# ygina/sidekick

Hardware: AMD Instinct MI355X
Metric: quACK encode identifiers/s (device-resident), u32 ids, threshold t=32 (higher is better)
Workload: dtype u32; 1 GPU; encode 1e+09 u32 ids per GPU at t=32, device-resident; ids_per_gpu=1000000000, global_ids=1000000000, threshold=32, bits=32, seed=0x5eed0002, parallelism=shard1, collectives=single

## Files before the change

### sidekick_amd/csrc/api.hip

```cpp
#include <string.h>

#include <algorithm>
#include <chrono>
#include <thread>
#include <vector>

#include "ctx.h"
#include "field.h"

using namespace qk;

#pragma clang diagnostic ignored "-Wunused-value"
#pragma clang diagnostic ignored "-Wunused-result"

namespace qk {

QK_WARM_KERNEL(api)

hipStream_t pick_stream(qk_ctx *ctx, void *stream) {
    (void)ctx;
    return (hipStream_t)stream;
}

int scratch_acquire(qk_ctx *ctx, hipStream_t s) {
// ... 336 lines not shown
template int root_test_begin<uint32_t>(qk_ctx *, const RtPlan<uint32_t> &, const uint32_t *, uint32_t,
                                       const uint32_t *, size_t, int, uint32_t, hipStream_t);
template int root_test_begin<uint64_t>(qk_ctx *, const RtPlan<uint64_t> &, const uint64_t *, uint32_t,
                                       const uint64_t *, size_t, int, uint64_t, hipStream_t);
template int root_test_finish<uint32_t>(qk_ctx *, const RtPlan<uint32_t> &, const uint32_t *, uint32_t,
                                        const uint32_t *, size_t, int, uint32_t, hipStream_t, std::vector<uint64_t> &,
                                        uint64_t &);
template int root_test_finish<uint64_t>(qk_ctx *, const RtPlan<uint64_t> &, const uint64_t *, uint32_t,
                                        const uint64_t *, size_t, int, uint64_t, hipStream_t, std::vector<uint64_t> &,
                                        uint64_t &);

template <typename T>
static int root_test_scan_k(qk_ctx *ctx, const T *coeffs, uint32_t d, const T *d_log, size_t n, int use_stop,
                            T stop_value, hipStream_t s, std::vector<uint64_t> &h, uint64_t &stop) {
    std::vector<T> r(d);
    uint32_t k = 0;
    int rc;
    if constexpr (sizeof(T) == 4) rc = qk_u32_roots(coeffs, d, r.data(), d, &k);
    else rc = qk_u64_roots(coeffs, d, r.data(), d, &k);
    if (rc) return rc;
    RtScanSet set;
    std::vector<T> tab;
    if (!rt_scan_table<T>(r.data(), k, set, tab, true) || set.words * sizeof(T) > RT_KTAB_BYTES) return 1;
    if (int e = ensure_hits(ctx, 4096, s)) return e;
    uint64_t *hs = ctx->h_small;
    if (!ctx->rt_bases_valid) {
        QK_HIP_TRY(hipMemsetAsync(ctx->d_small + SMALL_KT, 0, 4 * sizeof(uint64_t), s));
        ctx->rt_hbase = ctx->rt_sbase = 0;
    }
    if (!ctx->rt_slots_clean) {
        std::fill(hs + SMALL_HITPF, hs + SMALL_WORDS, ~0ull);
        hs[SMALL_OVF] = 0;
    }
    ctx->rt_slots_clean = false;
    const uint64_t gen = ++ctx->rt_gen;
    if (int e = launch_root_scan_k<T>(ctx, tab, set, d_log, n, use_stop, stop_value, ctx->d_hits,
                                      (uint64_t)ctx->hits_cap, ctx->d_small + SMALL_KT, ctx->h_small_dev + SMALL_NHITS,
                                      ctx->rt_hbase, ctx->rt_sbase, ctx->d_small + RT_DONE, gen, s)) {
        ctx->rt_bases_valid = false;
        return e;
    }
    ctx->rt_bases_valid = true;
    const volatile uint64_t *done = hs + SMALL_DONE;
    for (unsigned spin = 0;; ++spin) {
        if (*done == gen) break;
        if ((spin & 63) == 63) {
            const hipError_t q = hipStreamQuery(s);
            if (q != hipSuccess && q != hipErrorNotReady) {
                ctx->rt_bases_valid = false;
                return QK_E_HIP;
            }
            if (q == hipSuccess) {
                if (*done == gen) break;
                QK_HIP_TRY(hipMemsetAsync(ctx->d_small + RT_DONE, 0, (SMALL_DEV_WORDS - RT_DONE) * sizeof(uint64_t), s));
                break;
            }
        }
        if (spin >= 200000) std::this_thread::sleep_for(std::chrono::microseconds(5));
    }
    std::atomic_thread_fence(std::memory_order_acquire);
    if (hs[SMALL_OVF]) {
        ctx->rt_bases_valid = false;
        return 1;
    }
    uint64_t c = 0;
    while (c < SMALL_HITPF_N && hs[SMALL_HITPF + c] != ~0ull) ++c;
    uint64_t st = ~0ull, ns = 0;
    for (uint32_t q = 0; q < RT_NSTOP; ++q) {
        st = std::min(st, hs[SMALL_STOPS + q]);
        ns += hs[SMALL_STOPS + q] != ~0ull;
    }
    ctx->rt_hbase += c;
    ctx->rt_sbase += ns;
    h.assign(hs + SMALL_HITPF, hs + SMALL_HITPF + c);
    std::fill(hs + SMALL_HITPF, hs + SMALL_HITPF + c, ~0ull);
    std::fill(hs + SMALL_STOPS, hs + SMALL_WORDS, ~0ull);
    ctx->rt_slots_clean = true;
    std::sort(h.begin(), h.end());
    stop = use_stop ? std::min<uint64_t>(st, (uint64_t)n) : (uint64_t)n;
    return QK_OK;
}

template <typename T>
static int root_test_impl(qk_ctx *ctx, const T *coeffs, uint32_t d, const T *d_log, size_t n, int use_stop,
                          T stop_value, uint64_t *hits, size_t cap, size_t *n_hits, void *stream,
                          uint64_t *stop_index = nullptr) {
    if (!ctx || !n_hits || (d && !coeffs) || (n && !d_log)) return QK_E_INVAL;
    *n_hits = 0;
    if (stop_index) *stop_index = n;
    if (n == 0) return QK_OK;
    if (d == 0) {
        if (!stop_index || !use_stop) return QK_OK;
    }
    if (d > QK_MAX_THRESHOLD) return QK_E_THRESHOLD;
    if (!is_device_ptr(d_log)) return QK_E_INVAL;
    std::lock_guard<std::mutex> g(ctx->mu);
    QK_HIP_TRY(hipSetDevice(ctx->device));
    hipStream_t s = pick_stream(ctx, stream);
    std::vector<uint64_t> h;
    uint64_t stop = n;
    int ov = 1;
    if (ctx->knobs.rt_karg && rt_use_scan<T>(ctx, d, n)) {
        ov = root_test_scan_k<T>(ctx, coeffs, d, d_log, n, use_stop, stop_value, s, h, stop);
        if (ov < 0) return ov;
    }
    if (ov) {
        RtPlan<T> plan;
// ... 105 lines not shown
int qk_ctx_set_profiling(qk_ctx *ctx, int on) {
    if (!ctx) return QK_E_INVAL;
    std::lock_guard<std::mutex> g(ctx->mu);
    ctx->profiling = on != 0;
    return QK_OK;
}

int qk_ctx_kernel_stats(qk_ctx *ctx, double *total_ms, uint64_t *launches) {
    if (!ctx || !total_ms || !launches) return QK_E_INVAL;
    std::lock_guard<std::mutex> g(ctx->mu);
    double tot = 0;
    uint64_t cnt = 0;
    int rc = QK_OK;
    for (auto &pr : ctx->prof_pending) {
        if (hipEventSynchronize(pr.second) != hipSuccess) rc = QK_E_HIP;
        float ms = 0;
        if (hipEventElapsedTime(&ms, pr.first, pr.second) == hipSuccess) { tot += ms; ++cnt; }
        ctx->ev_pool.push_back(pr.first);
        ctx->ev_pool.push_back(pr.second);
    }
    ctx->prof_pending.clear();
    *total_ms = tot;
    *launches = cnt;
    return rc;
}

int qk_ctx_trim(qk_ctx *ctx) {
    if (!ctx) return QK_E_INVAL;
    std::lock_guard<std::mutex> g(ctx->mu);
    if (ctx->retired.empty()) return QK_OK;
    QK_HIP_TRY(hipSetDevice(ctx->device));
    int rc = QK_OK;
    for (void *r : ctx->retired)
        if (hipFree(r) != hipSuccess) rc = QK_E_HIP;
    ctx->retired.clear();
    return rc;
}

int qk_ctx_set_grid(qk_ctx *ctx, uint32_t blocks) {
    if (!ctx) return QK_E_INVAL;
    ctx->grid_override = blocks;
    return QK_OK;
}

int qk_ctx_set_knob(qk_ctx *ctx, const char *name, int64_t value) {
    if (!ctx || !name) return QK_E_INVAL;
    struct K {
        const char *name;
        int qk_knobs::*field;
        int64_t lo, hi;
    };
    static const K table[] = {
        {"grid_mult", &qk_knobs::grid_mult, 1, 8},
        {"flow_hist", &qk_knobs::flow_hist, 0, 1 << 20},
        {"flow_byslot", &qk_knobs::flow_byslot, 0, 2},
        {"root_test", &qk_knobs::root_test, 0, 2},
        {"comm_fault", &qk_knobs::comm_fault, 0, 1 << 20},
        {"comm_delay_ms", &qk_knobs::comm_delay_ms, 0, 600000},
        {"rt_karg", &qk_knobs::rt_karg, 0, 1},
    };
    for (const K &k : table)
        if (strcmp(k.name, name) == 0) {
            if (value < k.lo || value > k.hi) return QK_E_INVAL;
            std::lock_guard<std::mutex> g(ctx->mu);
            ctx->knobs.*(k.field) = (int)value;
            return QK_OK;
        }
    return QK_E_INVAL;
}

__global__ void k_clock_probe(uint64_t *out, uint64_t ticks) {
    const uint64_t c0 = __builtin_amdgcn_s_memtime(), r0 = __builtin_amdgcn_s_memrealtime();
    uint64_t c1, r1;
    do {
        __builtin_amdgcn_s_sleep(32);
        c1 = __builtin_amdgcn_s_memtime();
        r1 = __builtin_amdgcn_s_memrealtime();
    } while (r1 - r0 < ticks);
    if (threadIdx.x == 0) {
        out[0] = c1 - c0;
        out[1] = r1 - r0;
    }
}

int qk_clock_probe(qk_ctx *ctx, uint32_t microseconds, uint64_t *d_out, void *stream) {
    if (!ctx || !d_out || !microseconds || microseconds > 10000000u) return QK_E_INVAL;
    if (!is_device_ptr(d_out)) return QK_E_INVAL;
    QK_HIP_TRY(hipSetDevice(ctx->device));
    hipLaunchKernelGGL(k_clock_probe, dim3(1), dim3(64), 0, (hipStream_t)stream, d_out, (uint64_t)microseconds * 100);
    QK_HIP_TRY(hipGetLastError());
    return QK_OK;
}

int qk_host_alloc(size_t bytes, void **out) {
    if (!out) return QK_E_INVAL;
    if (hipHostMalloc(out, bytes, hipHostMallocDefault) != hipSuccess) { *out = nullptr; return QK_E_NOMEM; }
    return QK_OK;
}
int qk_host_free(void *p) {
    if (p && hipHostFree(p) != hipSuccess) return QK_E_HIP;
    return QK_OK;
}

int qk_u32_encode_device_async(qk_ctx *ctx, const uint32_t *d_ids, size_t n, uint32_t t, uint64_t *d_partial,
                               void *stream) {
    if (!ctx || !d_partial || (n && !d_ids)) return QK_E_INVAL;
// ... 157 lines not shown
```

### sidekick_amd/csrc/bsgs.h

```cpp
#pragma once
#include <hip/hip_runtime.h>
#include <stdint.h>

#include "field.h"

namespace qk {
namespace bsgs {

constexpr int BLOCK = 256;
constexpr int WAVES = BLOCK / 64;

__device__ __forceinline__ uint64_t shfl_xor_u64(uint64_t v, int m) {
    const uint32_t lo = __shfl_xor((int)(uint32_t)v, m, 64);
    const uint32_t hi = __shfl_xor((int)(uint32_t)(v >> 32), m, 64);
    return ((uint64_t)hi << 32) | lo;
}

#define QK_MAC4V(P0, P1, P2, P3)                                                                       \
    "v_mad_u64_u32 %0, " P0 ", %8, %9, %0\n\t"                                                         \
    "v_mad_u64_u32 %1, " P1 ", %8, %10, %1\n\t"                                                        \
    "v_mad_u64_u32 %2, " P2 ", %8, %11, %2\n\t"                                                        \
    "v_mad_u64_u32 %3, " P3 ", %8, %12, %3\n\t"                                                        \
    "v_addc_co_u32_e64 %4, " P0 ", %4, 0, " P0 "\n\t"                                                  \
    "v_addc_co_u32_e64 %5, " P1 ", %5, 0, " P1 "\n\t"                                                  \
// ... 576 lines not shown
            nxc = *pc;
        }
        four<C>(S, w, base, c, &xo);
        if constexpr (XO) {
            *po = xo;
            po += nthr;
        }
    }
    for (; it < tmax; ++it) {
        const uint4 w = nxt, c = nxc;
        const bool cur = p < vend;
        p += nthr;
        nxt = make_uint4(0, 0, 0, 0);
        if (p < vend) nxt = *p;
        if constexpr (XI) {
            pc += nthr;
            if (p < vend) nxc = *pc;
        }
        four<C>(S, w, base, c, &xo);
        if constexpr (XO) {
            if (cur) *po = xo;
            po += nthr;
        }
        (void)cur;
    }
    const uint64_t tail0 = h + (nbody << 2);
    const uint32_t tid = wave_s * 64u + __lane_id();
    gtid = (((uint64_t)gb_hi << 32) | gb_lo) + tid;
    {
        const bool in = gtid < h;
        uint32_t xn = 0;
        one<C>(S, in ? ids[gtid] : 0u, base, XI && in ? xin[gtid] : 0u, &xn);
        if (XO && in) xout[gtid] = xn;
    }
    {
        const bool in = gtid < n - tail0;
        uint32_t xn = 0;
        one<C>(S, in ? ids[tail0 + gtid] : 0u, base, XI && in ? xin[tail0 + gtid] : 0u, &xn);
        if (XO && in) xout[tail0 + gtid] = xn;
    }

    finish<C>(S, T, out, tid);
}

template <class C>
__device__ __forceinline__ void body(const uint32_t *__restrict__ ids, uint64_t n, uint32_t head, uint32_t T,
                                     uint64_t *__restrict__ partials, uint32_t base = 0,
                                     const uint32_t *xin = nullptr, uint32_t *xout = nullptr) {
    body_gen<C>(
        ids, n, head, T, (uint64_t)blockIdx.x * BLOCK + threadIdx.x, (uint64_t)gridDim.x * BLOCK,
        [=](uint32_t m, uint64_t s) { partials[(size_t)m * gridDim.x + blockIdx.x] = s; }, base, xin, xout);
}

}
}
```

### sidekick_amd/csrc/ctx.h

```cpp
#pragma once
#include <hip/hip_runtime.h>

#include <atomic>
#include <mutex>
#include <vector>

#include "quack_hip.h"

struct qk_knobs {
    int grid_mult = 3;
    int flow_hist = 32;
    int flow_byslot = 0;
    int root_test = 0;
    int comm_fault = 0;
    int rt_karg = 1;
    int comm_delay_ms = 0;
};

struct qk_ctx {
    int device = 0;
    int num_cus = 256;
    int max_threads_per_cu = 2048;
    uint32_t max_blocks_per_cu(uint32_t block) const { return (uint32_t)max_threads_per_cu / block; }
    hipStream_t stream = nullptr;
    hipStream_t copy_stream = nullptr;
    uint32_t grid_override = 0;
    qk_knobs knobs;

    void *d_scratch = nullptr;
    size_t scratch_bytes = 0;
    uint64_t *d_small = nullptr;
    uint64_t *h_small = nullptr;
    uint64_t *h_small_dev = nullptr;
    uint64_t rt_hbase = 0, rt_sbase = 0;
    bool rt_bases_valid = false;
    bool rt_slots_clean = false;
    int rt_occ_k[2] = {0, 0};
    uint64_t rt_gen = 0;
    uint64_t *d_hits = nullptr;
    size_t hits_cap = 0;

    void *d_flow[3] = {nullptr, nullptr, nullptr};
    size_t flow_bytes[3] = {0, 0, 0};
    size_t flow_hint = 0;
    void *h_items = nullptr;
    void *h_items_dev = nullptr;
    size_t h_items_bytes = 0;

    void *h_stage[2] = {nullptr, nullptr};
    void *d_stage[2] = {nullptr, nullptr};
    size_t stage_bytes = 0;
    hipEvent_t stage_ev[2] = {nullptr, nullptr};

    bool profiling = false;
    std::vector<std::pair<hipEvent_t, hipEvent_t>> prof_pending;
    std::vector<hipEvent_t> ev_pool;

    hipEvent_t scratch_ev = nullptr;
    bool scratch_ev_valid = false;
    hipEvent_t flow_ev[3] = {nullptr, nullptr, nullptr};
    uint64_t *h_flow = nullptr;

    std::vector<void *> retired;

    std::mutex mu;
};

#define QK_HIP_TRY(expr)                                                                           \
    do {                                                                                           \
        hipError_t _e = (expr);                                                                    \
        if (_e != hipSuccess) return QK_E_HIP;                                                     \
    } while (0)

namespace qk {

constexpr size_t SMALL_WORDS = 4096;
constexpr size_t RT_C = 4;
constexpr size_t SMALL_NHITS = 3072;
constexpr size_t SMALL_STOP = 3073;
constexpr size_t SMALL_OVF = 3074;
constexpr size_t SMALL_DONE = 3075;
constexpr size_t SMALL_HITPF = 3076;
constexpr uint32_t RT_NSTOP = 16;
constexpr size_t SMALL_STOPS = SMALL_WORDS - RT_NSTOP;
constexpr size_t SMALL_HITPF_N = SMALL_STOPS - SMALL_HITPF;
constexpr size_t RT_STOP0 = SMALL_STOPS - SMALL_NHITS;
constexpr size_t SMALL_KT = SMALL_WORDS - 8;
constexpr uint32_t RT_DONE_GROUPS = 32;
constexpr size_t RT_DONE = SMALL_WORDS;
constexpr size_t SMALL_DEV_WORDS = RT_DONE + 16 * (RT_DONE_GROUPS + 1);

#define QK_WARM_KERNEL(name)                                                                                     \
    __global__ void k_warm_##name(int *p) {                                                                      \
        if (p) p[threadIdx.x] = 0;                                                                               \
    }                                                                                                            \
    int warm_##name(hipStream_t s) {                                                                             \
        hipLaunchKernelGGL(k_warm_##name, dim3(1), dim3(64), 0, s, nullptr);                                     \
        return hipGetLastError() == hipSuccess ? QK_OK : QK_E_HIP;                                               \
    }
int warm_api(hipStream_t s);
int warm_encode(hipStream_t s);
int warm_decode(hipStream_t s);
int warm_packets(hipStream_t s);
int warm_flows(hipStream_t s);
int warm_segments(hipStream_t s);
int warm_comm(hipStream_t s);

hipStream_t pick_stream(qk_ctx *ctx, void *stream);
int scratch_acquire(qk_ctx *ctx, hipStream_t s);
int scratch_release(qk_ctx *ctx, hipStream_t s);
int ensure_scratch(qk_ctx *ctx, size_t bytes, hipStream_t s);
int ensure_hits(qk_ctx *ctx, size_t cap, hipStream_t s);
int ensure_flow(qk_ctx *ctx, int which, size_t bytes, hipStream_t s);
int ensure_stage(qk_ctx *ctx, size_t bytes);
int ensure_items(qk_ctx *ctx, size_t bytes);
bool is_device_ptr(const void *p);
hipEvent_t prof_begin(qk_ctx *ctx, hipStream_t s);
void prof_end(qk_ctx *ctx, hipStream_t s, hipEvent_t begin);

int launch_encode_u32(qk_ctx *ctx, const uint32_t *d_ids, size_t n, uint32_t t, uint64_t *d_partial,
                      hipStream_t s);
int launch_encode_u64(qk_ctx *ctx, const uint64_t *d_ids, size_t n, uint32_t t, uint64_t *d_partial,
                      hipStream_t s);
int launch_encode_u32_acc(qk_ctx *ctx, const uint32_t *d_ids, size_t n, uint32_t t,
                          uint64_t *d_partial, hipStream_t s);
int launch_encode_u64_acc(qk_ctx *ctx, const uint64_t *d_ids, size_t n, uint32_t t,
                          uint64_t *d_partial, hipStream_t s);

int launch_root_test_u32(qk_ctx *ctx, const uint32_t *d_c, uint32_t d, const uint32_t *log, size_t n,
                         int use_stop, uint32_t stop_value, uint64_t *hits, uint64_t cap, uint64_t *counters,
                         hipStream_t s);
int launch_finalize_powers_u32(const uint64_t *partials, uint32_t nblocks, uint32_t T, uint64_t *out,
                               hipStream_t s);
bool rt64_use_bsgs(const qk_ctx *ctx, uint32_t d);
constexpr uint32_t RT_SCAN_MAXD = 256;
size_t rt64_bsgs_table(const uint64_t *coeffs, uint32_t d, uint64_t *out);
int launch_root_test_u64(qk_ctx *ctx, const uint64_t *d_c, uint32_t d, const uint64_t *log, size_t n,
                         int use_stop, uint64_t stop_value, uint64_t *hits, uint64_t cap, uint64_t *counters,
                         hipStream_t s);

struct RtScanSet {
    uint32_t S = 1, words = 0, m1 = 1, m2 = 1, shift = 28;
};
// ... 30 lines not shown
```

### sidekick_amd/csrc/encode.hip

```cpp
#include "ctx.h"
#include "field.h"
#include "bsgs.h"
#include "bsgs64.h"

#ifndef QK_BSGS_SG_T32
#define QK_BSGS_SG_T32 8
#endif
#ifndef QK_BSGS_ROW0
#define QK_BSGS_ROW0 1
#endif
#ifndef QK_BSGS_FOLD
#define QK_BSGS_FOLD 1
#endif

namespace qk {

QK_WARM_KERNEL(encode)

constexpr int BLOCK = 256;
constexpr int WAVES = BLOCK / 64;

__device__ __forceinline__ uint64_t shfl_xor_u64(uint64_t v, int m) {
    const uint32_t lo = __shfl_xor((int)(uint32_t)v, m, 64);
    const uint32_t hi = __shfl_xor((int)(uint32_t)(v >> 32), m, 64);
    return ((uint64_t)hi << 32) | lo;
}


template <int K>
__device__ __forceinline__ void chain32(uint64_t (&acc)[K], uint32_t start, uint32_t step) {
    const uint32_t step5 = times5_32(step);
    uint64_t t = start;
#pragma unroll
    for (int k = 0; k < K; ++k) {
        acc[k] += t;
        if (k + 1 < K) t = tstep32p(t, step, step5, 0u);
    }
}

template <int K>
__device__ __forceinline__ void chain32x4(uint64_t (&acc)[K], uint4 w) {
    const uint32_t x0 = canon32(w.x), x1 = canon32(w.y), x2 = canon32(w.z), x3 = canon32(w.w);
    const uint32_t f0 = times5_32(x0), f1 = times5_32(x1), f2 = times5_32(x2), f3 = times5_32(x3);
    uint64_t t0 = x0, t1 = x1, t2 = x2, t3 = x3;
#pragma unroll
    for (int k = 0; k < K; ++k) {
        acc[k] += t0;
        acc[k] += t1;
        acc[k] += t2;
        acc[k] += t3;
        if (k + 1 < K) {
            t0 = tstep32p(t0, x0, f0, 0u);
            t1 = tstep32p(t1, x1, f1, 0u);
            t2 = tstep32p(t2, x2, f2, 0u);
            t3 = tstep32p(t3, x3, f3, 0u);
        }
    }
}

template <int NB, int NA, int SG, int PRIO = 1>
__global__ __launch_bounds__(BLOCK, (NB * NA == 32 ? 5 : NB * NA > 64 ? 2 : NB * NA > 40 ? 3 : 4)) void k_encode_u32_bsgs(const uint32_t *__restrict__ ids,
                                                                                  uint64_t n, uint32_t head,
                                                                                  uint32_t T,
                                                                                  uint64_t *__restrict__ partials) {
    bsgs::body<bsgs::Cfg<NB, NA, SG, QK_BSGS_ROW0, QK_BSGS_FOLD, false, false, 0, false, PRIO ? 4 : 0>>(ids, n, head,
                                                                                                        T, partials);
}


template <int SG, int PRIO = 1>
__global__ __launch_bounds__(BLOCK, 2) void k_encode_u32_bsgs_x80(const uint32_t *__restrict__ ids, uint64_t n,
                                                                 uint32_t head, uint32_t T,
                                                                 uint64_t *__restrict__ partials,
                                                                 const uint32_t *xin,
                                                                 uint32_t *xout) {
    (void)xin;
    bsgs::body<bsgs::Cfg<8, 10, SG, 1, 1, false, false, 2, false, PRIO ? 4 : 0>>(ids, n, head, T, partials, 0, nullptr,
                                                                                 xout);
}

template <int NA, int SG, int XC = 0, int PRIO = 1>
__global__ __launch_bounds__(BLOCK, (NA > 6 ? 2 : NA > 5 ? 3 : 4)) void k_encode_u32_bsgs_off(
    const uint32_t *__restrict__ ids, uint64_t n, uint32_t head, uint32_t T, uint32_t base,
    uint64_t *__restrict__ partials, const uint32_t *xin, uint32_t *xout) {
    bsgs::body<bsgs::Cfg<8, NA, SG, 1, 1, false, true, XC, false, PRIO ? 4 : 0>>(ids, n, head, T, partials, base, xin,
                                                                                 xout);
}

template <int G>
__device__ __forceinline__ void group_powers32(uint32_t x, int j, uint32_t &start, uint32_t &step) {
    uint32_t b = x, r = 1;
    const uint32_t e = (uint32_t)j + 1;
#pragma unroll
    for (int bit = 0; (1 << bit) <= G; ++bit) {
        const uint32_t rb = mul32_lazy(r, b);
        r = ((e >> bit) & 1) ? rb : r;
        if ((1 << bit) < G) b = mul32_lazy(b, b);
    }
    start = r;
    step = canon32(b);
}

template <int G, int K, typename Fold>
__device__ __forceinline__ void block_store(const uint64_t (&acc)[K], uint32_t T, uint64_t *partials,
                                            uint64_t *sm, Fold fold) {
    const int lane = threadIdx.x & 63, wave = threadIdx.x >> 6;
#pragma unroll
    for (int k = 0; k < K; ++k) {
        uint64_t v = fold(acc[k]);
#pragma unroll
        for (int off = 32; off >= G; off >>= 1) v += shfl_xor_u64(v, off);
        if (lane < G) sm[wave * (G * K) + lane + k * G] = v;
    }
    __syncthreads();
    for (uint32_t m = threadIdx.x; m < T; m += BLOCK) {
        uint64_t s = 0;
#pragma unroll
        for (int w = 0; w < WAVES; ++w) s += sm[w * (G * K) + m];
        partials[(size_t)m * gridDim.x + blockIdx.x] = s;
    }
}
// ... 358 lines not shown
                                                                          uint64_t *xout) {
    (void)head;
    bsgs64::body<10, F ? 3 : 0, 16, 0, 0, false, true, 1, 2, bsgs64::NB, F ? 3 : 0>(ids, n, T, partials, 0, nullptr,
                                                                                 xout);
}

template <int NA, int XC = 0, int F = 1>
__global__ __launch_bounds__(bsgs64::BLOCK, 4) void k_encode_u64_bsgs_off(const uint64_t *__restrict__ ids,
                                                                          uint64_t n, uint32_t head, uint32_t T,
                                                                          uint32_t base,
                                                                          uint64_t *__restrict__ partials,
                                                                          const uint64_t *xin,
                                                                          uint64_t *xout) {
    (void)head;
    bsgs64::body<NA, F ? 3 : 0, 16, 0, 0, true, true, 1, XC, bsgs64::NB, F ? 3 : 0>(ids, n, T, partials, base, xin,
                                                                                     xout);
}

template <typename KernelT>
static uint32_t grid_for(qk_ctx *ctx, KernelT kern, uint64_t units, uint32_t per_block, int mult = 0) {
    if (ctx->grid_override) return ctx->grid_override;
    int occ = 0;
    if (hipOccupancyMaxActiveBlocksPerMultiprocessor(&occ, kern, BLOCK, 0) != hipSuccess || occ < 1) occ = 1;
    const uint64_t full = (uint64_t)ctx->num_cus * (uint64_t)occ * (uint64_t)(mult > 0 ? mult : ctx->knobs.grid_mult);
    uint64_t need = (units + per_block - 1) / per_block;
    if (need < 1) need = 1;
    return (uint32_t)(need < full ? need : full);
}

static uint32_t grid_cap(const qk_ctx *ctx, uint64_t units, uint32_t per_block, int mult = 0) {
    if (ctx->grid_override) return ctx->grid_override;
    const uint64_t full = (uint64_t)ctx->num_cus * (uint64_t)ctx->max_blocks_per_cu(BLOCK) *
                          (uint64_t)(mult > 0 ? mult : ctx->knobs.grid_mult);
    uint64_t need = (units + per_block - 1) / per_block;
    if (need < 1) need = 1;
    return (uint32_t)(need < full ? need : full);
}

template <typename IdT, typename KernelT, typename FinT>
static int run_encode(qk_ctx *ctx, KernelT kern, FinT fin, uint32_t GK, uint32_t words_per_power,
                      const IdT *d_ids, size_t n, uint32_t head, uint32_t T, uint64_t units,
                      uint32_t per_block, uint64_t *d_partial, int accumulate, hipStream_t s, int mult = 0) {
    const uint32_t nb = grid_for(ctx, kern, units, per_block, mult);
    const size_t need = (size_t)nb * words_per_power * GK * sizeof(uint64_t);
    int rc = ensure_scratch(ctx, need, s);
    if (rc) return rc;
    uint64_t *partials = (uint64_t *)ctx->d_scratch;
    rc = scratch_acquire(ctx, s);
    if (rc) return rc;
    hipEvent_t e0 = prof_begin(ctx, s);
    hipLaunchKernelGGL(kern, dim3(nb), dim3(BLOCK), 0, s, d_ids, (uint64_t)n, head, T, partials);
    prof_end(ctx, s, e0);
    QK_HIP_TRY(hipGetLastError());
    hipLaunchKernelGGL(fin, dim3(T), dim3(BLOCK), 0, s, partials, nb, T, d_ids, (uint64_t)n, d_partial,
                       accumulate);
    QK_HIP_TRY(hipGetLastError());
    return scratch_release(ctx, s);
}

int launch_finalize_powers_u32(const uint64_t *partials, uint32_t nblocks, uint32_t T, uint64_t *out,
                               hipStream_t s) {
    hipLaunchKernelGGL(k_finalize_u32_pass, dim3(T), dim3(BLOCK), 0, s, partials, nblocks, T,
                       (const uint32_t *)nullptr, (uint64_t)0, out, (uint64_t *)nullptr, 0);
    return hipGetLastError() == hipSuccess ? QK_OK : QK_E_HIP;
}

template <int KIND, class KernelT>
static int run_pass(qk_ctx *ctx, KernelT kern, uint32_t GK, const uint32_t *d_ids, size_t n,
                    uint32_t head, uint32_t Tp, uint32_t base, uint64_t *out, uint64_t *meta, int acc,
                    hipStream_t s, const uint32_t *xin = nullptr, uint32_t *xout = nullptr) {
    const uint32_t nb = grid_for(ctx, kern, (n + 3) / 4, BLOCK, 1);
    if (int rc = ensure_scratch(ctx, (size_t)nb * GK * sizeof(uint64_t), s)) return rc;
    uint64_t *partials = (uint64_t *)ctx->d_scratch;
    if (int rc = scratch_acquire(ctx, s)) return rc;
    hipEvent_t e0 = prof_begin(ctx, s);
    if constexpr (KIND == 1)
        hipLaunchKernelGGL(kern, dim3(nb), dim3(BLOCK), 0, s, d_ids, (uint64_t)n, head, Tp, base, partials, xin,
                           xout);
    else if constexpr (KIND == 2)
        hipLaunchKernelGGL(kern, dim3(nb), dim3(BLOCK), 0, s, d_ids, (uint64_t)n, head, Tp, partials, xin, xout);
    else
        hipLaunchKernelGGL(kern, dim3(nb), dim3(BLOCK), 0, s, d_ids, (uint64_t)n, head, Tp, partials);
    prof_end(ctx, s, e0);
    QK_HIP_TRY(hipGetLastError());
    hipLaunchKernelGGL(k_finalize_u32_pass, dim3(Tp), dim3(BLOCK), 0, s, partials, nb, Tp, d_ids, (uint64_t)n, out,
                       meta, acc);
    QK_HIP_TRY(hipGetLastError());
    return scratch_release(ctx, s);
}


static int enc32_passes_chunk(qk_ctx *ctx, const uint32_t *ids, size_t n, uint32_t head, uint32_t T, uint64_t *out,
                              int acc, hipStream_t s) {
    const uint32_t npass = T <= 80 ? 0 : (T - 80 + 47) / 48;
    uint32_t *xc = nullptr;
    if (npass >= 1) {
        const uint32_t nbmax = grid_cap(ctx, (n + 3) / 4, BLOCK, 1);
        const size_t poff = ((size_t)nbmax * 80 * sizeof(uint64_t) + 255) & ~(size_t)255;
        if (ensure_scratch(ctx, poff + 16 + (size_t)n * 4, s) == QK_OK)
            xc = (uint32_t *)((char *)ctx->d_scratch + poff + ((uintptr_t)ids & 15));
    }
    uint32_t pass = 0;
    for (uint32_t base = 0; base < T; ++pass) {
        const uint32_t Tp = std::min<uint32_t>(base == 0 ? 80 : 48, T - base);
        uint64_t *meta = base == 0 ? out + T : nullptr;
        const int xcm = !xc ? 0 : (pass > 0 ? 1 : 0) | (pass < npass ? 2 : 0);
// ... 195 lines not shown
        return run_encode<uint64_t>(ctx, k_encode_u64_gn<G, K>, k_finalize_u64, G * K, 2, ids, n, head, T,
                                    n, BLOCK / G, out, acc, s);
}

template <int G>
static int enc64_g(qk_ctx *ctx, int K, const uint64_t *ids, size_t n, uint32_t head, uint32_t T, uint64_t *out,
                   int acc, hipStream_t s) {
    if constexpr (G == 1) {
        switch (K) {
        case 1: return enc64_gk<1, 1>(ctx, ids, n, head, T, out, acc, s);
        case 2: return enc64_gk<1, 2>(ctx, ids, n, head, T, out, acc, s);
        case 4: return enc64_gk<1, 4>(ctx, ids, n, head, T, out, acc, s);
        case 8: return enc64_gk<1, 8>(ctx, ids, n, head, T, out, acc, s);
        case 12: return enc64_gk<1, 12>(ctx, ids, n, head, T, out, acc, s);
        case 16: return enc64_gk<1, 16>(ctx, ids, n, head, T, out, acc, s);
        case 20: return enc64_gk<1, 20>(ctx, ids, n, head, T, out, acc, s);
        case 24: return enc64_gk<1, 24>(ctx, ids, n, head, T, out, acc, s);
        case 32: return enc64_gk<1, 32>(ctx, ids, n, head, T, out, acc, s);
        case 40: return enc64_gk<1, 40>(ctx, ids, n, head, T, out, acc, s);
        }
    } else {
        switch (K) {
        case 12: return enc64_gk<G, 12>(ctx, ids, n, head, T, out, acc, s);
        case 16: return enc64_gk<G, 16>(ctx, ids, n, head, T, out, acc, s);
        case 20: return enc64_gk<G, 20>(ctx, ids, n, head, T, out, acc, s);
        case 24: return enc64_gk<G, 24>(ctx, ids, n, head, T, out, acc, s);
        case 32: return enc64_gk<G, 32>(ctx, ids, n, head, T, out, acc, s);
        case 40: return enc64_gk<G, 40>(ctx, ids, n, head, T, out, acc, s);
        }
    }
    return QK_E_THRESHOLD;
}

static void choose_gk(uint32_t T, int kmax, const int *kg1, int nkg1, const int *kgn, int nkgn, int &G, int &K) {
    G = 1;
    while ((T + G - 1) / G > (uint32_t)kmax) G *= 2;
    const uint32_t kneed = (T + G - 1) / G;
    const int *ks = G == 1 ? kg1 : kgn;
    const int nk = G == 1 ? nkg1 : nkgn;
    K = ks[nk - 1];
    for (int i = 0; i < nk; ++i)
        if ((uint32_t)ks[i] >= kneed) { K = ks[i]; break; }
}


static int enc32(qk_ctx *ctx, const uint32_t *ids, size_t n, uint32_t T, uint64_t *out, int acc, hipStream_t s) {
    if (T == 0 || T > QK_MAX_THRESHOLD) return QK_E_THRESHOLD;
    const uintptr_t a = (uintptr_t)ids;
    if (a & 3) return QK_E_INVAL;
    const uint32_t head = (uint32_t)(((16 - (a & 15)) & 15) / 4);
    if (n >= (1ull << 40)) return QK_E_INVAL;
    const uint64_t min_grid = ctx->grid_override ? ctx->grid_override : (uint64_t)ctx->num_cus;
    const bool sc_ok = n / (4ull * BLOCK * min_grid) < (1ull << 24) - 2;
#define QK_BSGS(NB_, NA_, G_)                                                                                 \
    run_encode<uint32_t>(ctx, k_encode_u32_bsgs<NB_, NA_, G_, 1>, k_finalize_u32, NB_ * NA_, 1, ids, n, head, T, \
                         (n + 3) / 4, BLOCK, out, acc, s, NB_ * NA_ > 48 ? 1 : 0)
    if (T >= 5 && T <= 8 && sc_ok) return QK_BSGS(4, 2, 1);
    if (T >= 9 && T <= 12) return sc_ok ? QK_BSGS(4, 3, 3) : QK_BSGS(4, 3, 0);
    if (T >= 13 && T <= 16) return sc_ok ? QK_BSGS(4, 4, 4) : QK_BSGS(4, 4, 0);
    if (sc_ok) {
        if (T >= 17 && T <= 20) return QK_BSGS(4, 5, 5);
        if (T >= 21 && T <= 24) return QK_BSGS(4, 6, 6);
        if (T >= 25 && T <= 28) return QK_BSGS(4, 7, 7);
        if (T >= 29 && T <= 30) return QK_BSGS(6, 5, 5);
        if (T >= 31 && T <= 32) return QK_BSGS(8, 4, QK_BSGS_SG_T32);
        if (T >= 33 && T <= 36) return QK_BSGS(6, 6, 6);
        if (T >= 37 && T <= 40) return QK_BSGS(8, 5, 10);
        if (T >= 41 && T <= 42) return QK_BSGS(6, 7, 7);
        if (T >= 43 && T <= 48) return QK_BSGS(8, 6, 12);
        if (T >= 49 && T <= 56) return QK_BSGS(8, 7, 14);
        if (T >= 57 && T <= 64) return QK_BSGS(8, 8, 16);
        if (T >= 65 && T <= 72) return QK_BSGS(8, 9, 14);
        if (T >= 73 && T <= 80) return QK_BSGS(8, 10, 16);
        if (T > 80) return enc32_passes(ctx, ids, n, head, T, out, acc, s);
    } else {
        if (T >= 17 && T <= 24) return QK_BSGS(6, 4, 0);
        if (T >= 25 && T <= 32) return QK_BSGS(8, 4, 0);
    }
#undef QK_BSGS
    int G, K;
    choose_gk(T, 32, K32_G1, 10, K32_GN, 4, G, K);
    switch (G) {
    case 1: return enc32_g<1>(ctx, K, ids, n, head, T, out, acc, s);
    case 2: return enc32_g<2>(ctx, K, ids, n, head, T, out, acc, s);
    case 4: return enc32_g<4>(ctx, K, ids, n, head, T, out, acc, s);
    case 8: return enc32_g<8>(ctx, K, ids, n, head, T, out, acc, s);
    case 16: return enc32_g<16>(ctx, K, ids, n, head, T, out, acc, s);
    case 32: return enc32_g<32>(ctx, K, ids, n, head, T, out, acc, s);
    }
    return QK_E_THRESHOLD;
}

static int enc64(qk_ctx *ctx, const uint64_t *ids, size_t n, uint32_t T, uint64_t *out, int acc, hipStream_t s) {
    if (T == 0 || T > QK_MAX_THRESHOLD) return QK_E_THRESHOLD;
    const uintptr_t a = (uintptr_t)ids;
    if (a & 7) return QK_E_INVAL;
    const uint32_t head = (uint32_t)(((16 - (a & 15)) & 15) / 8);
    const uint64_t min_grid64 = ctx->grid_override ? ctx->grid_override : (uint64_t)ctx->num_cus;
    const bool bsgs_ok = n / min_grid64 < (1ull << 30);
    if (T >= 14 && T <= 80 && bsgs_ok) {
#define QK_BSGS64(NA_, SG_)                                                                           \
    run_encode<uint64_t>(ctx, k_encode_u64_bsgs<NA_, SG_, 1>, k_finalize_u64, 8 * NA_, 2, ids, n, head, T,   \
                         (n + bsgs64::BLOCK - 1) / bsgs64::BLOCK, 1, out, acc, s)
#define QK_BSGS64_4(NA_)                                                                              \
    run_encode<uint64_t>(ctx, k_encode_u64_bsgs4<NA_, 1>, k_finalize_u64, 4 * NA_, 2, ids, n, head, T,      \
                         (n + bsgs64::BLOCK - 1) / bsgs64::BLOCK, 1, out, acc, s)
        if (T <= 36) switch ((T + 3) / 4) {
            case 4: return QK_BSGS64_4(4);
            case 5: return QK_BSGS64_4(5);
            case 7: return QK_BSGS64_4(7);
            case 9: return QK_BSGS64_4(9);
            default: break;
            }
#undef QK_BSGS64_4
        switch ((T + 7) / 8) {
        case 2: return QK_BSGS64(2, 16);
        case 3: return QK_BSGS64(3, 16);
        case 4: return QK_BSGS64(4, 16);
        case 5: return QK_BSGS64(5, 16);
        case 6: return QK_BSGS64(6, 16);
        case 7: return QK_BSGS64(7, 16);
        case 8: return QK_BSGS64(8, 16);
        case 9: return QK_BSGS64(9, 16);
        default: return QK_BSGS64(10, 14);
        }
#undef QK_BSGS64
    }
    if (T > 80 && bsgs_ok) return enc64_passes(ctx, ids, n, head, T, out, acc, s);
    int G, K;
    choose_gk(T, 40, K64_G1, 10, K64_GN, 6, G, K);
    switch (G) {
    case 1: return enc64_g<1>(ctx, K, ids, n, head, T, out, acc, s);
// ... 27 lines not shown
```

Before: 455.0 billion identifiers/s.

## Add dynamic chunk-claiming encode kernel with atomic work counters for u32 BSGS

Adds a dynamic work-distribution variant of the u32 BSGS encode in which each wave claims fixed-size chunks of ids through atomic counters spread over eight regions, replacing the static grid-stride split. Loads go through buffer resources and are software-prefetched one group ahead, with the next chunk claimed while the current one is processed. The goal is to even out load imbalance and tail effects across CUs. In exchange it adds an atomic per chunk, per-context counter bases that grow monotonically across calls, and hand-written asm that clobbers fixed registers.

```diff
diff --git a/sidekick_amd/csrc/api.hip b/sidekick_amd/csrc/api.hip
--- a/sidekick_amd/csrc/api.hip
+++ b/sidekick_amd/csrc/api.hip
@@ -412,7 +412,7 @@
             }
             if (q == hipSuccess) {
                 if (*done == gen) break;
-                QK_HIP_TRY(hipMemsetAsync(ctx->d_small + RT_DONE, 0, (SMALL_DEV_WORDS - RT_DONE) * sizeof(uint64_t), s));
+                QK_HIP_TRY(hipMemsetAsync(ctx->d_small + RT_DONE, 0, RT_DONE_WORDS * sizeof(uint64_t), s));
                 break;
             }
         }
@@ -624,6 +624,7 @@
     };
     static const K table[] = {
         {"grid_mult", &qk_knobs::grid_mult, 1, 8},
+        {"enc_dyn", &qk_knobs::enc_dyn, 0, 1},
         {"flow_hist", &qk_knobs::flow_hist, 0, 1 << 20},
         {"flow_byslot", &qk_knobs::flow_byslot, 0, 2},
         {"root_test", &qk_knobs::root_test, 0, 2},
diff --git a/sidekick_amd/csrc/bsgs.h b/sidekick_amd/csrc/bsgs.h
--- a/sidekick_amd/csrc/bsgs.h
+++ b/sidekick_amd/csrc/bsgs.h
@@ -652,5 +652,119 @@
         [=](uint32_t m, uint64_t s) { partials[(size_t)m * gridDim.x + blockIdx.x] = s; }, base, xin, xout);
 }
 
-}
-}
+#ifndef QK_DYN_CH
+#define QK_DYN_CH 16
+#endif
+constexpr int DYN_CH = QK_DYN_CH;
+constexpr uint32_t DYN_GROUPS = DYN_CH * 64;
+
+__device__ __forceinline__ uint64_t claim_chunk(unsigned long long *ctr, uint64_t cbase) {
+    uint32_t lo, hi;
+    asm volatile("v_mov_b32_e32 v6, 1\n\t"
+                 "v_mov_b32_e32 v7, 0\n\t"
+                 "s_mov_b64 s[58:59], exec\n\t"
+                 "s_mov_b64 exec, 1\n\t"
+                 "global_atomic_add_x2 v[6:7], v7, v[6:7], %[ctr] sc0\n\t"
+                 "s_mov_b64 exec, s[58:59]\n\t"
+                 "s_waitcnt vmcnt(0)\n\t"
+                 "v_readfirstlane_b32 %[lo], v6\n\t"
+                 "v_readfirstlane_b32 %[hi], v7"
+                 : [lo] "=s"(lo), [hi] "=s"(hi)
+                 : [ctr] "s"(ctr)
+                 : "v6", "v7", "s58", "s59", "memory");
+    return (((uint64_t)hi << 32) | lo) - cbase;
+}
+
+typedef uint32_t u32x4_t __attribute__((ext_vector_type(4)));
+__device__ __forceinline__ __amdgpu_buffer_rsrc_t chunk_rsrc(const char *vb, uint64_t g) {
+    return __builtin_amdgcn_make_buffer_rsrc(const_cast<char *>(vb + g * 16u), 0, (int)(DYN_GROUPS * 16u),
+                                             0x00020000);
+}
+__device__ __forceinline__ uint4 chunk_group(__amdgpu_buffer_rsrc_t rs, uint32_t slot, uint32_t j) {
+    const u32x4_t w = __builtin_amdgcn_raw_buffer_load_b128(rs, (int)slot, (int)(j * 1024u), 0);
+    return make_uint4(w.x, w.y, w.z, w.w);
+}
+
+constexpr int DYN_NCTR = 8;
+constexpr int DYN_CTR_STRIDE = 544;
+struct DynArgs {
+    unsigned long long *ctr;
+    uint64_t region;
+    uint64_t base[DYN_NCTR];
+};
+__host__ __device__ inline uint64_t dyn_region_len(uint64_t nchunks, uint64_t region, uint32_t k) {
+    const uint64_t lo = (uint64_t)k * region;
+    return lo >= nchunks ? 0 : (nchunks - lo < region ? nchunks - lo : region);
+}
+
+template <class C>
+__device__ __forceinline__ void body_dyn(const uint32_t *__restrict__ ids, uint64_t n, uint32_t head, uint32_t T,
+                                         uint64_t *__restrict__ partials, const DynArgs &da) {
+    static_assert(!C::OFF && C::XC == 0, "dynamic chunks: plain single-pass configurations");
+    Acc<C::NB, C::NA, C::ROWS> S;
+    clear<C>(S);
+    const uint32_t wave_s = (uint32_t)__builtin_amdgcn_readfirstlane((int)(threadIdx.x >> 6));
+    const uint64_t h = head < n ? head : n;
+    const uint64_t nbody = (n - h) >> 2;
+    const uint64_t nchunks = nbody / DYN_GROUPS;
+    const char *vb = reinterpret_cast<const char *>(ids + h);
+    const uint32_t slot = __lane_id() * 16u;
+    constexpr uint64_t NONE = ~0ull;
+    uint32_t k = blockIdx.x % (uint32_t)DYN_NCTR, failed = 0;
+    bool rest_mine = false;
+    auto claim = [&]() -> uint64_t {
+        while (failed < (uint32_t)DYN_NCTR) {
+            const uint64_t idx = claim_chunk(da.ctr + (size_t)k * DYN_CTR_STRIDE, da.base[k]);
+            const uint64_t len = dyn_region_len(nchunks, da.region, k);
+            if (idx < len) return (uint64_t)k * da.region + idx;
+            if (k == 0 && idx == len) rest_mine = true;
+            k = k + 1 == (uint32_t)DYN_NCTR ? 0u : k + 1;
+            ++failed;
+        }
+        return NONE;
+    };
+    uint4 nxt = make_uint4(0, 0, 0, 0);
+    uint64_t cur = claim();
+    __amdgpu_buffer_rsrc_t rs = chunk_rsrc(vb, 0);
+    if (cur != NONE) {
+        rs = chunk_rsrc(vb, cur * DYN_GROUPS);
+        nxt = chunk_group(rs, slot, 0);
+    }
+    while (cur != NONE) {
+        const uint64_t next = claim();
+        for (uint32_t j = 1; j < (uint32_t)DYN_CH; ++j) {
+            const uint4 w = nxt;
+            nxt = chunk_group(rs, slot, j);
+            four<C>(S, w, 0);
+        }
+        const uint4 w = nxt;
+        if (next != NONE) {
+            rs = chunk_rsrc(vb, next * DYN_GROUPS);
+            nxt = chunk_group(rs, slot, 0);
+        }
+        four<C>(S, w, 0);
+        cur = next;
+    }
+    if (rest_mine) {
+        const uint32_t lane = __lane_id();
+        const uint32_t rest = (uint32_t)(nbody - nchunks * DYN_GROUPS);
+        rs = chunk_rsrc(vb, nchunks * DYN_GROUPS);
+        nxt = make_uint4(0, 0, 0, 0);
+        if (lane < rest) nxt = chunk_group(rs, slot, 0);
+        for (uint32_t j = 0; j * 64u < rest; ++j) {
+            const uint4 w = nxt;
+            nxt = make_uint4(0, 0, 0, 0);
+            if ((j + 1) * 64u + lane < rest) nxt = chunk_group(rs, slot, j + 1);
+            four<C>(S, w, 0);
+        }
+        const uint64_t tail0 = h + (nbody << 2);
+        one<C>(S, lane < h ? ids[lane] : 0u);
+        one<C>(S, lane < n - tail0 ? ids[tail0 + lane] : 0u);
+    }
+    finish<C>(
+        S, T, [=](uint32_t m, uint64_t s) { partials[(size_t)m * gridDim.x + blockIdx.x] = s; },
+        wave_s * 64u + __lane_id());
+}
+
+}
+}
diff --git a/sidekick_amd/csrc/ctx.h b/sidekick_amd/csrc/ctx.h
--- a/sidekick_amd/csrc/ctx.h
+++ b/sidekick_amd/csrc/ctx.h
@@ -9,6 +9,7 @@
 
 struct qk_knobs {
     int grid_mult = 3;
+    int enc_dyn = 1;
     int flow_hist = 32;
     int flow_byslot = 0;
     int root_test = 0;
@@ -39,6 +40,7 @@
     uint64_t rt_gen = 0;
     uint64_t *d_hits = nullptr;
     size_t hits_cap = 0;
+    uint64_t enc_claim_base[8] = {0, 0, 0, 0, 0, 0, 0, 0};
 
     void *d_flow[3] = {nullptr, nullptr, nullptr};
     size_t flow_bytes[3] = {0, 0, 0};
@@ -88,7 +90,10 @@
 constexpr size_t SMALL_KT = SMALL_WORDS - 8;
 constexpr uint32_t RT_DONE_GROUPS = 32;
 constexpr size_t RT_DONE = SMALL_WORDS;
-constexpr size_t SMALL_DEV_WORDS = RT_DONE + 16 * (RT_DONE_GROUPS + 1);
+constexpr size_t RT_DONE_WORDS = 16 * (RT_DONE_GROUPS + 1);
+constexpr size_t ENC_CLAIM = RT_DONE + RT_DONE_WORDS;
+constexpr size_t ENC_CLAIM_WORDS = 8 * 544;
+constexpr size_t SMALL_DEV_WORDS = ENC_CLAIM + ENC_CLAIM_WORDS;
 
 #define QK_WARM_KERNEL(name)                                                                                     \
     __global__ void k_warm_##name(int *p) {                                                                      \
diff --git a/sidekick_amd/csrc/encode.hip b/sidekick_amd/csrc/encode.hip
--- a/sidekick_amd/csrc/encode.hip
+++ b/sidekick_amd/csrc/encode.hip
@@ -67,6 +67,13 @@
                                                                                                         T, partials);
 }
 
+template <int NB, int NA, int SG, int PRIO = 1>
+__global__ __launch_bounds__(BLOCK, (NB * NA == 32 ? 5 : NB * NA > 64 ? 2 : NB * NA > 40 ? 3 : 4)) void k_encode_u32_bsgs_dyn(
+    const uint32_t *__restrict__ ids, uint64_t n, uint32_t head, uint32_t T, uint64_t *__restrict__ partials,
+    const bsgs::DynArgs da) {
+    bsgs::body_dyn<bsgs::Cfg<NB, NA, SG, QK_BSGS_ROW0, QK_BSGS_FOLD, false, false, 0, false, PRIO ? 4 : 0>>(
+        ids, n, head, T, partials, da);
+}
 
 template <int SG, int PRIO = 1>
 __global__ __launch_bounds__(BLOCK, 2) void k_encode_u32_bsgs_x80(const uint32_t *__restrict__ ids, uint64_t n,
@@ -531,6 +538,36 @@
     hipLaunchKernelGGL(kern, dim3(nb), dim3(BLOCK), 0, s, d_ids, (uint64_t)n, head, T, partials);
     prof_end(ctx, s, e0);
     QK_HIP_TRY(hipGetLastError());
+    hipLaunchKernelGGL(fin, dim3(T), dim3(BLOCK), 0, s, partials, nb, T, d_ids, (uint64_t)n, d_partial,
+                       accumulate);
+    QK_HIP_TRY(hipGetLastError());
+    return scratch_release(ctx, s);
+}
+
+static_assert((size_t)bsgs::DYN_NCTR * bsgs::DYN_CTR_STRIDE <= ENC_CLAIM_WORDS &&
+                  bsgs::DYN_NCTR == sizeof(qk_ctx::enc_claim_base) / sizeof(uint64_t),
+              "ctx.h: room for the dynamic encode's counters and their bases");
+template <typename KernelT, typename FinT>
+static int run_encode_dyn(qk_ctx *ctx, KernelT kern, FinT fin, uint32_t GK, const uint32_t *d_ids, size_t n,
+                          uint32_t head, uint32_t T, uint64_t *d_partial, int accumulate, hipStream_t s) {
+    const uint32_t nb = grid_for(ctx, kern, ((uint64_t)n + 3) / 4, BLOCK, 1);
+    int rc = ensure_scratch(ctx, (size_t)nb * GK * sizeof(uint64_t), s);
+    if (rc) return rc;
+    uint64_t *partials = (uint64_t *)ctx->d_scratch;
+    rc = scratch_acquire(ctx, s);
+    if (rc) return rc;
+    const uint64_t h = head < n ? head : n;
+    const uint64_t nchunks = ((n - h) >> 2) / bsgs::DYN_GROUPS;
+    bsgs::DynArgs da;
+    da.ctr = (unsigned long long *)(ctx->d_small + ENC_CLAIM);
+    da.region = (nchunks + bsgs::DYN_NCTR - 1) / bsgs::DYN_NCTR;
+    for (int k = 0; k < bsgs::DYN_NCTR; ++k) da.base[k] = ctx->enc_claim_base[k];
+    hipEvent_t e0 = prof_begin(ctx, s);
+    hipLaunchKernelGGL(kern, dim3(nb), dim3(BLOCK), 0, s, d_ids, (uint64_t)n, head, T, partials, da);
+    prof_end(ctx, s, e0);
+    QK_HIP_TRY(hipGetLastError());
+    for (int k = 0; k < bsgs::DYN_NCTR; ++k)
+        ctx->enc_claim_base[k] += bsgs::dyn_region_len(nchunks, da.region, (uint32_t)k) + (uint64_t)nb * WAVES;
     hipLaunchKernelGGL(fin, dim3(T), dim3(BLOCK), 0, s, partials, nb, T, d_ids, (uint64_t)n, d_partial,
                        accumulate);
     QK_HIP_TRY(hipGetLastError());
@@ -832,12 +869,17 @@
     if (n >= (1ull << 40)) return QK_E_INVAL;
     const uint64_t min_grid = ctx->grid_override ? ctx->grid_override : (uint64_t)ctx->num_cus;
     const bool sc_ok = n / (4ull * BLOCK * min_grid) < (1ull << 24) - 2;
-#define QK_BSGS(NB_, NA_, G_)                                                                                 \
+    const bool dyn = ctx->knobs.enc_dyn != 0 && n < (1ull << 32);
+#define QK_BSGS_STATIC(NB_, NA_, G_)                                                                          \
     run_encode<uint32_t>(ctx, k_encode_u32_bsgs<NB_, NA_, G_, 1>, k_finalize_u32, NB_ * NA_, 1, ids, n, head, T, \
                          (n + 3) / 4, BLOCK, out, acc, s, NB_ * NA_ > 48 ? 1 : 0)
+#define QK_BSGS(NB_, NA_, G_)                                                                                 \
+    (dyn ? run_encode_dyn(ctx, k_encode_u32_bsgs_dyn<NB_, NA_, G_, 1>, k_finalize_u32, NB_ * NA_, ids, n, head, T, \
+                          out, acc, s)                                                                        \
+         : QK_BSGS_STATIC(NB_, NA_, G_))
     if (T >= 5 && T <= 8 && sc_ok) return QK_BSGS(4, 2, 1);
-    if (T >= 9 && T <= 12) return sc_ok ? QK_BSGS(4, 3, 3) : QK_BSGS(4, 3, 0);
-    if (T >= 13 && T <= 16) return sc_ok ? QK_BSGS(4, 4, 4) : QK_BSGS(4, 4, 0);
+    if (T >= 9 && T <= 12) return sc_ok ? QK_BSGS(4, 3, 3) : QK_BSGS_STATIC(4, 3, 0);
+    if (T >= 13 && T <= 16) return sc_ok ? QK_BSGS(4, 4, 4) : QK_BSGS_STATIC(4, 4, 0);
     if (sc_ok) {
         if (T >= 17 && T <= 20) return QK_BSGS(4, 5, 5);
         if (T >= 21 && T <= 24) return QK_BSGS(4, 6, 6);
@@ -854,10 +896,11 @@
         if (T >= 73 && T <= 80) return QK_BSGS(8, 10, 16);
         if (T > 80) return enc32_passes(ctx, ids, n, head, T, out, acc, s);
     } else {
-        if (T >= 17 && T <= 24) return QK_BSGS(6, 4, 0);
-        if (T >= 25 && T <= 32) return QK_BSGS(8, 4, 0);
+        if (T >= 17 && T <= 24) return QK_BSGS_STATIC(6, 4, 0);
+        if (T >= 25 && T <= 32) return QK_BSGS_STATIC(8, 4, 0);
     }
 #undef QK_BSGS
+#undef QK_BSGS_STATIC
     int G, K;
     choose_gk(T, 32, K32_G1, 10, K32_GN, 4, G, K);
     switch (G) {
```

New measurement: 481.1 billion identifiers/s (median of 6 runs). 1.06x the previous value.
